# intel/oim

Hardware: AMD Instinct MI355X
Metric: 4KiB_randread_IOPS (higher is better)
Workload: dtype uint8

## Files before the change

native/include/hipstore/engine.h:

```cpp

#pragma once

#include <cstdint>
#include <functional>
#include <map>
#include <string>
#include <vector>

#include "hipstore/bdev.h"

namespace hipstore {

bool gpu_available();
int gpu_device_count();
std::string gpu_pci_address(int device);

BdevPtr create_hbm_bdev(const std::string& name, uint64_t block_size,
                        uint64_t num_blocks, int device,
                        bool persistent = false);

uint64_t persistent_stat(int which);

std::map<std::string, long long> persistent_probe(int device, int flags);

std::map<std::string, long long> persistent_kernel_probe(int device,
                                                         int variant);

std::pair<uint64_t, uint64_t> hbm_info(int device);

void* alloc_pinned(size_t bytes);
void free_pinned(void* ptr);

int hbm_copy_sync(Bdev* src, uint64_t src_offset, Bdev* dst,
                  uint64_t dst_offset, uint64_t length);

struct DiffStats {
  uint64_t granules = 0;
  uint64_t mismatched = 0;
  std::vector<uint64_t> first_mismatches;
};
int bdev_diff_sync(Bdev* a, uint64_t a_offset, Bdev* b, uint64_t b_offset,
                   uint64_t length, uint32_t granule, uint32_t max_report,
                   std::vector<uint64_t>* bitmap_out, DiffStats* stats);

uint64_t bdev_common_length(Bdev* a, uint64_t a_offset, Bdev* b,
                            uint64_t b_offset, uint32_t granule);

int bdev_copy_marked_sync(Bdev* src, uint64_t src_offset, Bdev* dst,
                          uint64_t dst_offset, uint64_t length,
                          uint32_t granule,
                          const std::vector<uint64_t>& bitmap,
                          uint64_t* copied = nullptr);

using PackSink =
    std::function<int(const uint8_t* data, uint64_t first_rank, uint64_t count)>;
int bdev_pack_marked_sync(Bdev* src, uint64_t src_offset, uint64_t length,
                          uint32_t granule,
                          const std::vector<uint64_t>& bitmap,
                          uint64_t staging_bytes, const PackSink& sink,
                          uint64_t* packed = nullptr);

using UnpackSource =
    std::function<int(uint8_t* data, uint64_t first_rank, uint64_t count)>;
int bdev_unpack_marked_sync(Bdev* dst, uint64_t dst_offset, uint64_t length,
// ... 16 lines not shown
  uint64_t granules = 0;
  uint64_t calls = 0;
};
int marked_copy_probe(Bdev* src, uint32_t granule,
                      const std::vector<uint64_t>& bitmap, int mode,
                      uint64_t ring_bytes, uint64_t staging_bytes,
                      MarkedCopyProbe* out);

int bdev_read_sync(Bdev* bdev, uint64_t offset, void* buf, uint64_t len);
int bdev_write_sync(Bdev* bdev, uint64_t offset, const void* buf, uint64_t len);
int bdev_fill_sync(Bdev* bdev, uint64_t offset, uint8_t value, uint64_t len);

class IoQueue {
 public:
  struct Op {
    IoOp op = IoOp::kRead;
    uint64_t offset = 0;
    uint64_t length = 0;
    uint8_t fill = 0;
    std::string payload;
  };
  struct Result {
    int status = kIoFailed;
    bool has_data = false;
    std::string data;
  };

  explicit IoQueue(BdevPtr bdev);

  const char* kind() const;

  std::vector<Result> run(const std::vector<Op>& ops);

  ~IoQueue();
  IoQueue(const IoQueue&) = delete;
  IoQueue& operator=(const IoQueue&) = delete;

 private:
  uint8_t* acquire_arena(uint64_t bytes);

  BdevPtr bdev_;
  std::shared_ptr<IoChannel> channel_;
  uint8_t* arena_ = nullptr;
  uint64_t arena_capacity_ = 0;
  std::vector<void*> retired_;
  bool busy_ = false;
};

struct PerfResult {
  double seconds = 0;
  uint64_t io_count = 0;
  double iops = 0;
  double throughput_mbps = 0;
  double lat_avg_us = 0;
  double lat_p50_us = 0;
  double lat_p90_us = 0;
  double lat_p99_us = 0;
  double lat_p999_us = 0;
  double lat_max_us = 0;
};

PerfResult run_bdevperf(Bdev* bdev, const std::string& workload,
                        uint32_t io_size, uint32_t queue_depth,
                        int num_queues, double seconds,
                        uint64_t max_ios = 0);

class PerfSession {
 public:
  PerfSession(BdevPtr bdev, std::string workload, uint32_t io_size,
              uint32_t queue_depth, int num_queues);
  ~PerfSession();

  PerfResult step(uint64_t total_ios);

 private:
  struct Impl;
  std::unique_ptr<Impl> impl_;
};

// ... 2 lines not shown
```

native/src/gpu.hip:

```cpp

#include <hip/hip_runtime.h>
#include <pthread.h>
#include <sched.h>
#include <unistd.h>
#include <stdlib.h>

#include <algorithm>
#include <atomic>
#include <chrono>
#include <condition_variable>
#include <cstring>
#include <deque>
#include <functional>
#include <map>
#include <mutex>
#include <random>
#include <set>
#include <stdexcept>
#include <thread>
#include <utility>
#include <vector>

#include "gpu_internal.h"
#include "hipstore/engine.h"

namespace hipstore {


namespace {

constexpr uint32_t kTileBytes = 4096;
constexpr uint32_t kRingSlots = 1 << 16;
constexpr uint32_t kMaxBatchTiles = kRingSlots / 4;

struct BlockDesc {
  const uint8_t* src;
  uint8_t* dst;
  uint32_t bytes;
  uint32_t fill;
};
static_assert(sizeof(BlockDesc) == 24, "persistent engine reads 3 x u64");

__global__ __launch_bounds__(kWavesPerWg * 64) void k_copy_blocks(
    const BlockDesc* __restrict__ descs, uint32_t n) {
  __shared__ __attribute__((aligned(16))) uint8_t lds_raw[kWavesPerWg * kTileBytes];
  const uint32_t wave = threadIdx.x >> 6;
  const uint32_t lane = threadIdx.x & 63;
  const uint32_t idx = blockIdx.x * kWavesPerWg + wave;
  if (idx >= n) return;
  const BlockDesc d = descs[idx];
  float4* lds = reinterpret_cast<float4*>(lds_raw + wave * kTileBytes);
  const uint32_t n16 = d.bytes >> 4;
  if (d.src != nullptr) {
    const float4* __restrict__ src = reinterpret_cast<const float4*>(d.src);
#pragma unroll 4
    for (uint32_t i = lane; i < n16; i += 64) lds[i] = src[i];
  } else {
// ... 446 lines not shown
  if (hipDeviceGetPCIBusId(bus_id, sizeof(bus_id), device) != hipSuccess) {
    return "";
  }
  std::string s(bus_id);
  std::transform(s.begin(), s.end(), s.begin(), ::tolower);
  return s;
}

std::pair<uint64_t, uint64_t> hbm_info(int device) {
  if (!gpu_available() || device < 0 || device >= gpu_device_count()) {
    return {0, 0};
  }
  if (hipSetDevice(device) != hipSuccess) return {0, 0};
  size_t free_bytes = 0;
  size_t total_bytes = 0;
  if (hipMemGetInfo(&free_bytes, &total_bytes) != hipSuccess) return {0, 0};
  return {total_bytes, free_bytes};
}

void* alloc_pinned(size_t bytes) {
  if (!gpu_available()) return malloc(bytes);
  void* p = nullptr;
  HIP_CHECK(hipHostMalloc(&p, bytes, hipHostMallocMapped));
  return p;
}

void free_pinned(void* ptr) {
  if (ptr == nullptr) return;
  if (!gpu_available()) {
    free(ptr);
    return;
  }
  (void)hipHostFree(ptr);
}


namespace {

class HbmChannelBase : public IoChannel {
 public:
  virtual void enqueue(IoRequest req, int status) = 0;
  virtual int poll() = 0;
  virtual const char* kind_name() const = 0;
};

inline HbmChannelBase* hbm_channel(IoChannel* ch) {
  return static_cast<HbmChannelBase*>(ch);
}

uint8_t* buf_device(uint8_t* host) {
  void* dev = nullptr;
  hipError_t err = hipHostGetDevicePointer(&dev, host, 0);
  if (err != hipSuccess) {
    throw std::runtime_error(
        "hipstore: I/O buffer is not pinned host memory (use alloc_pinned)");
  }
  return static_cast<uint8_t*>(dev);
}

inline uint32_t tile_count(uint64_t length) {
  return static_cast<uint32_t>((length + kTileBytes - 1) / kTileBytes);
}

void fill_desc(BlockDesc& d, const IoRequest& req, uint8_t* base,
               uint64_t done, uint32_t bytes) {
  if (req.op == IoOp::kRead) {
    d.src = base + req.offset + done;
    d.dst = buf_device(static_cast<uint8_t*>(req.buffer) + done);
  } else if (req.op == IoOp::kWrite) {
    d.src = buf_device(static_cast<uint8_t*>(req.buffer) + done);
    d.dst = base + req.offset + done;
  } else {
    d.src = nullptr;
    d.dst = base + req.offset + done;
  }
  d.bytes = bytes;
  d.fill = req.fill;
}

struct PendingIo {
  IoRequest req;
  int status;
};

struct InflightBatch {
  hipEvent_t event = nullptr;
  uint32_t slots = 0;
  std::vector<std::pair<IoCompletion, int>> completions;
};

class HbmChannel : public HbmChannelBase {
 public:
  HbmChannel(int device, uint8_t* base, uint64_t size)
      : base_(base), size_(size) {
    HIP_CHECK(hipSetDevice(device));
    HIP_CHECK(hipStreamCreateWithFlags(&stream_, hipStreamNonBlocking));
    HIP_CHECK(hipHostMalloc(reinterpret_cast<void**>(&ring_),
                            kRingSlots * sizeof(BlockDesc), hipHostMallocMapped));
    ring_dev_ = device_view(ring_);
    device_ = device;
  }

  ~HbmChannel() override {
// ... 56 lines not shown
    if (n > 0) {
      const uint32_t first = ring_head_;
      const uint32_t grid = (n + kWavesPerWg - 1) / kWavesPerWg;
      hipLaunchKernelGGL(k_copy_blocks, dim3(grid), dim3(kWavesPerWg * 64), 0,
                         stream_, ring_dev_ + first, n);
    }
    hipEvent_t event = get_event();
    HIP_CHECK(hipEventRecord(event, stream_));
    ring_head_ = (ring_head_ + n) % kRingSlots;
    used_slots_ += n;
    inflight_.push_back(InflightBatch{event, n, std::move(completions)});
  }

  int retire(bool wait) {
    int completed = 0;
    while (!inflight_.empty()) {
      InflightBatch& batch = inflight_.front();
      hipError_t st = wait ? hipEventSynchronize(batch.event)
                           : hipEventQuery(batch.event);
      if (st == hipErrorNotReady) break;
      if (st != hipSuccess) throw std::runtime_error("hip event failure");
      for (auto& [cb, status] : batch.completions) {
        if (cb) cb(status);
        ++completed;
      }
      used_slots_ -= batch.slots;
      event_pool_.push_back(batch.event);
      inflight_.pop_front();
    }
    return completed;
  }

  void expand(const IoRequest& req, uint32_t* slot) {
    uint64_t done = 0;
    while (done < req.length) {
      const uint32_t bytes = static_cast<uint32_t>(
          std::min<uint64_t>(kTileBytes, req.length - done));
      fill_desc(ring_[*slot], req, base_, done, bytes);
      ++*slot;
      done += bytes;
    }
  }

  hipEvent_t get_event() {
    if (!event_pool_.empty()) {
      hipEvent_t e = event_pool_.back();
      event_pool_.pop_back();
      return e;
    }
    hipEvent_t e = nullptr;
    HIP_CHECK(hipEventCreateWithFlags(&e, hipEventDisableTiming));
    return e;
  }

  uint8_t* base_;
  [[maybe_unused]] uint64_t size_;
  int device_ = 0;
  hipStream_t stream_ = nullptr;
  BlockDesc* ring_ = nullptr;
  BlockDesc* ring_dev_ = nullptr;
  uint32_t ring_head_ = 0;
  uint32_t used_slots_ = 0;
  std::vector<PendingIo> pending_;
  std::deque<InflightBatch> inflight_;
  std::vector<hipEvent_t> event_pool_;
};

class ServiceRingChannel : public HbmChannelBase {
 public:
  static constexpr uint32_t kRing = 32768;

  void enqueue(IoRequest req, int status) override {
    if (status != kIoOk) {
      immediate_.emplace_back(std::move(req.on_complete), status);
      return;
    }
    if (req.op == IoOp::kFlush) {
      flushes_.push_back({tail_, std::move(req.on_complete)});
      return;
    }
    pending_.push_back(std::move(req));
    drain_pending();
  }

  int poll() override {
    int completed = 0;
    if (!immediate_.empty()) {
      auto batch = std::move(immediate_);
      immediate_.clear();
      for (auto& [cb, status] : batch) {
        if (cb) cb(status);
        ++completed;
      }
    }
    const uint64_t retired_from = completed_;
    while (completed_ < tail_) {
// ... 54 lines not shown
    (void)hipHostFree(sq_);
    (void)hipHostFree(const_cast<unsigned long long*>(sq_tail_));
    (void)hipHostFree(const_cast<unsigned long long*>(cq_));
  }

  void delete_unfired() {
    std::set<IoState*> leftovers(desc_io_.begin(), desc_io_.end());
    for (IoState* state : leftovers) delete state;
  }

  BlockDesc* sq_ = nullptr;
  volatile unsigned long long* sq_tail_ = nullptr;
  volatile unsigned long long* cq_ = nullptr;
  uint64_t tail_ = 0;
  uint64_t completed_ = 0;
  std::chrono::steady_clock::time_point last_progress_{};

 private:
  struct IoState {
    IoCompletion cb;
    uint32_t remaining;
    int status;
  };

  bool has_capacity(uint32_t tiles) const {
    return tail_ - completed_ + tiles <= kRing;
  }

  void drain_pending() {
    while (!pending_.empty()) {
      IoRequest& req = pending_.front();
      const uint32_t tiles = tile_count(req.length);
      if (!has_capacity(tiles)) return;
      auto* state = new IoState{std::move(req.on_complete), tiles, kIoOk};
      uint64_t done = 0;
      uint64_t t = tail_;
      while (done < req.length) {
        const uint32_t bytes = static_cast<uint32_t>(
            std::min<uint64_t>(kTileBytes, req.length - done));
        fill_desc(sq_[t % kRing], req, base_, done, bytes);
        desc_io_[t % kRing] = state;
        ++t;
        done += bytes;
      }
      tail_ = t;
      __atomic_store_n(const_cast<unsigned long long*>(sq_tail_), tail_,
                       __ATOMIC_RELEASE);
      pending_.pop_front();
    }
  }

  uint8_t* base_;
  std::vector<IoState*> desc_io_;
  std::deque<IoRequest> pending_;
  std::deque<std::pair<uint64_t, IoCompletion>> flushes_;
  std::vector<std::pair<IoCompletion, int>> immediate_;
};

inline std::atomic<int> g_per_queue_channels[64];
inline int per_queue_channel_cap() {
  static const int cap = [] {
    const char* env = getenv("HIPSTORE_PERQ_CAP");
    return env ? atoi(env) : 18;
  }();
  return cap;
}

inline bool fallback_is_shared() {
  static const bool shared = [] {
    const char* env = getenv("HIPSTORE_FALLBACK");
    return env == nullptr || strcmp(env, "batched") != 0;
  }();
  return shared;
}

inline uint32_t batch_tiles_env() {
  const char* env = getenv("HIPSTORE_BATCH_TILES");
  const int v = env ? atoi(env) : 2;
  return static_cast<uint32_t>(
      std::min(std::max(v, 1), static_cast<int>(kMaxRunTiles)));
}

class HbmPersistentChannel : public ServiceRingChannel {
 public:
  static constexpr uint32_t kIdleSpins = 500000;

// ... 568 lines not shown
  req.fill = value;
  return run_sync(bdev, std::move(req));
}


IoQueue::IoQueue(BdevPtr bdev)
    : bdev_(std::move(bdev)), channel_(bdev_->get_channel()) {}

const char* IoQueue::kind() const {
  if (bdev_->device_base() == nullptr) return "cpu";
  return hbm_channel(channel_.get())->kind_name();
}

std::vector<IoQueue::Result> IoQueue::run(const std::vector<Op>& ops) {
  constexpr uint64_t kAlign = 64;
  std::vector<uint64_t> region(ops.size(), 0);
  uint64_t arena_bytes = kAlign;
  for (size_t i = 0; i < ops.size(); ++i) {
    if (ops[i].op != IoOp::kRead && ops[i].op != IoOp::kWrite) continue;
    region[i] = arena_bytes;
    arena_bytes += (ops[i].length + kAlign - 1) / kAlign * kAlign + kAlign;
  }
  uint8_t* arena = acquire_arena(arena_bytes);
  for (size_t i = 0; i < ops.size(); ++i) {
    if (ops[i].op == IoOp::kWrite && ops[i].length > 0) {
      memcpy(arena + region[i], ops[i].payload.data(), ops[i].length);
    } else if (ops[i].op == IoOp::kRead) {
      memset(arena + region[i], 0xDB, ops[i].length);
    }
  }

  struct RunState {
    std::vector<int> status;
    size_t remaining = 0;
  };
  auto state = std::make_shared<RunState>();
  state->status.assign(ops.size(), kIoFailed);
  state->remaining = ops.size();

  busy_ = true;
  for (size_t i = 0; i < ops.size(); ++i) {
    IoRequest req;
    req.op = ops[i].op;
    req.offset = ops[i].offset;
    req.length = ops[i].length;
    req.fill = ops[i].fill;
    if (req.op == IoOp::kRead || req.op == IoOp::kWrite) {
      req.buffer = arena + region[i];
    }
    req.on_complete = [state, i](int status) {
      state->status[i] = status;
      --state->remaining;
    };
    bdev_->submit(channel_.get(), std::move(req));
  }
  const auto deadline = std::chrono::steady_clock::now() +
                        std::chrono::duration<double>(sync_io_timeout_s());
  while (state->remaining > 0) {
    bdev_->poll(channel_.get());
    if (state->remaining > 0 &&
        std::chrono::steady_clock::now() > deadline) {
      dump_engine_stats("IoQueue timeout");
      throw std::runtime_error(
          "IoQueue: " + std::to_string(state->remaining) + " of " +
          std::to_string(ops.size()) + " requests still outstanding after " +
          std::to_string(sync_io_timeout_s()) + " s");
    }
  }

  std::vector<Result> results(ops.size());
  for (size_t i = 0; i < ops.size(); ++i) {
    results[i].status = state->status[i];
    if (ops[i].op == IoOp::kRead && state->status[i] == kIoOk) {
      results[i].has_data = true;
      results[i].data.assign(reinterpret_cast<const char*>(arena + region[i]),
                             ops[i].length);
    }
  }
  busy_ = false;
  return results;
}

uint8_t* IoQueue::acquire_arena(uint64_t bytes) {
  if (busy_) {
    arena_ = nullptr;
    arena_capacity_ = 0;
    retired_.clear();
    busy_ = false;
  }
  if (bytes > arena_capacity_) {
    if (arena_ != nullptr) retired_.push_back(arena_);
    arena_ = nullptr;
    arena_capacity_ = 0;
    void* p = alloc_pinned(bytes);
    if (p == nullptr) throw std::runtime_error("IoQueue: arena allocation");
    arena_ = static_cast<uint8_t*>(p);
    arena_capacity_ = bytes;
  }
  return arena_;
}

IoQueue::~IoQueue() {
  channel_.reset();
  if (busy_) return;
  for (void* p : retired_) free_pinned(p);
  free_pinned(arena_);
}


namespace {

struct LatHist {
// ... 361 lines not shown
  im.cv.notify_all();
  {
    const auto step_deadline =
        std::chrono::duration<double>(2 * sync_io_timeout_s() + 30.0);
    std::unique_lock<std::mutex> lock(im.mutex);
    const bool done = im.cv.wait_for(lock, step_deadline, [&] {
      for (auto& st : im.stats) {
        if (st.done_epoch < this_epoch) return false;
      }
      return true;
    });
    if (!done) {
      dump_engine_stats("perf-session step timeout");
      throw std::runtime_error("perf session: step timed out (wedged queue)");
    }
  }
  const double elapsed = std::chrono::duration<double>(clock::now() - t0).count();

  PerfResult result;
  result.seconds = elapsed;
  LatHist total;
  bool failed = false;
  for (auto& st : im.stats) {
    result.io_count += st.ios;
    failed |= st.failed;
    st.lat.merge_into(total);
  }
  if (failed) throw std::runtime_error("perf session: I/O failures");
  result.iops = result.io_count / elapsed;
  result.throughput_mbps =
      result.io_count * static_cast<double>(im.io_size) / elapsed / 1e6;
  total.fill_result(&result);
  return result;
}

std::map<std::string, long long> persistent_probe(int device, int flags) {
  std::map<std::string, long long> r;
  const bool use_atomics = flags & 1;
  const bool pre_memcpy = flags & 2;
  const bool do_rmw = flags & 4;
  const bool big_grid = flags & 8;
  const bool do_fence = flags & 16;
  r["flags"] = flags;
  HIP_CHECK(hipSetDevice(device));
  hipStream_t stream = nullptr;
  hipStream_t util = nullptr;
  HIP_CHECK(hipStreamCreateWithFlags(&stream, hipStreamNonBlocking));
  HIP_CHECK(hipStreamCreateWithFlags(&util, hipStreamNonBlocking));
  void* p_tail = nullptr;
  void* p_hb = nullptr;
  void* p_cq = nullptr;
  HIP_CHECK(hipHostMalloc(&p_tail, 8, hipHostMallocMapped));
  HIP_CHECK(hipHostMalloc(&p_hb, 8, hipHostMallocMapped));
  HIP_CHECK(hipHostMalloc(&p_cq, 16, hipHostMallocMapped));
  auto* tail = static_cast<volatile unsigned long long*>(p_tail);
  auto* hb = static_cast<volatile unsigned long long*>(p_hb);
  auto* cq = static_cast<volatile unsigned long long*>(p_cq);
  *tail = 0;
  *hb = 0;
  cq[0] = 0;
  cq[1] = 0;
  unsigned long long* dev_words = nullptr;
  HIP_CHECK(hipMalloc(reinterpret_cast<void**>(&dev_words), 24));
  HIP_CHECK(hipMemset(dev_words, 0, 24));
  HIP_CHECK(hipStreamSynchronize(nullptr));
  ProbeCtl ctl;
// ... 178 lines not shown
```

native/src/pybind.cpp:

```cpp

#include <pybind11/functional.h>
#include <pybind11/pybind11.h>
#include <pybind11/stl.h>

#include <cstring>
#include <optional>
#include <stdexcept>

#include "hipstore/bdev.h"
#include "hipstore/composite.h"
#include "hipstore/crc32c.h"
#include "hipstore/delta.h"
#include "hipstore/engine.h"
#include "hipstore/fingerprint.h"
#include "hipstore/nvmf.h"
#include "hipstore/rados.h"
#include "hipstore/vhost_master.h"

namespace py = pybind11;
using namespace hipstore;

namespace {

py::bytes bdev_read_py(Bdev& bdev, uint64_t offset, uint64_t length) {
  void* bounce = alloc_pinned(length);
  int status = bdev_read_sync(&bdev, offset, bounce, length);
  if (status != kIoOk) {
    free_pinned(bounce);
    throw std::runtime_error("bdev read failed: status " + std::to_string(status));
  }
  py::bytes out(static_cast<const char*>(bounce), length);
  free_pinned(bounce);
  return out;
}

void bdev_write_py(Bdev& bdev, uint64_t offset, py::buffer data) {
  py::buffer_info info = data.request();
  const uint64_t length = static_cast<uint64_t>(info.size) * info.itemsize;
  void* bounce = alloc_pinned(length);
  memcpy(bounce, info.ptr, length);
  int status = bdev_write_sync(&bdev, offset, bounce, length);
  free_pinned(bounce);
  if (status != kIoOk) {
    throw std::runtime_error("bdev write failed: status " + std::to_string(status));
  }
}

void bdev_fill_py(Bdev& bdev, uint64_t offset, int value, uint64_t length) {
  int status = bdev_fill_sync(&bdev, offset, static_cast<uint8_t>(value), length);
  if (status != kIoOk) {
    throw std::runtime_error("bdev fill failed: status " + std::to_string(status));
  }
}

IoQueue::Op io_op_from_tuple(const py::tuple& t) {
  if (t.empty()) throw std::invalid_argument("IoQueue: empty op tuple");
  const std::string name = t[0].cast<std::string>();
  IoQueue::Op op;
  if (name == "read" && t.size() == 3) {
    op.op = IoOp::kRead;
    op.offset = t[1].cast<uint64_t>();
    op.length = t[2].cast<uint64_t>();
  } else if (name == "write" && t.size() == 3) {
    op.op = IoOp::kWrite;
    op.offset = t[1].cast<uint64_t>();
    py::buffer_info info = t[2].cast<py::buffer>().request();
    op.payload.assign(static_cast<const char*>(info.ptr),
                      static_cast<size_t>(info.size) * info.itemsize);
    op.length = op.payload.size();
  } else if (name == "fill" && t.size() == 4) {
    op.op = IoOp::kFill;
    op.offset = t[1].cast<uint64_t>();
    op.length = t[2].cast<uint64_t>();
    op.fill = static_cast<uint8_t>(t[3].cast<int>());
  } else if (name == "flush" && t.size() == 1) {
    op.op = IoOp::kFlush;
  } else {
    throw std::invalid_argument("IoQueue: unknown op tuple '" + name + "'");
// ... 105 lines not shown
  }
  if (status == kIoOk) return;
  const std::string text = std::string(what) + ": " + error + " (status " +
                           std::to_string(status) + ")";
  if (status == kIoInvalid) throw std::invalid_argument(text);
  throw std::runtime_error(text);
}

}

PYBIND11_MODULE(_hipstore, m) {
  m.doc() = "MI355X hipstore data-path core (HBM bdevs, LDS-staged block I/O)";

  m.def("gpu_available", &gpu_available);
  m.def("gpu_device_count", &gpu_device_count);
  m.def("gpu_pci_address", &gpu_pci_address, py::arg("device"));

  py::class_<Bdev, BdevPtr>(m, "Bdev")
      .def_property_readonly("name", &Bdev::name)
      .def_property_readonly("product_name", &Bdev::product_name)
      .def_property_readonly("uuid", &Bdev::uuid)
      .def_property_readonly("block_size", &Bdev::block_size)
      .def_property_readonly("num_blocks", &Bdev::num_blocks)
      .def_property_readonly("size_bytes", &Bdev::size_bytes)
      .def("resize",
           [](hipstore::Bdev& b, uint64_t num_blocks) {
             return b.resize(num_blocks);
           },
           py::arg("num_blocks"))
      .def("read", &bdev_read_py, py::arg("offset"), py::arg("length"),
           py::call_guard<py::gil_scoped_release>())
      .def("write", &bdev_write_py, py::arg("offset"), py::arg("data"))
      .def("fill", &bdev_fill_py, py::arg("offset"), py::arg("value"),
           py::arg("length"), py::call_guard<py::gil_scoped_release>());

  m.def("create_malloc_bdev", &create_malloc_bdev, py::arg("name"),
        py::arg("block_size"), py::arg("num_blocks"));
  m.def("create_hbm_bdev", &create_hbm_bdev, py::arg("name"),
        py::arg("block_size"), py::arg("num_blocks"), py::arg("device") = 0,
        py::arg("persistent") = false);
  m.def("create_file_bdev", &create_file_bdev, py::arg("name"),
        py::arg("path"), py::arg("block_size") = 512);
  m.def("create_striped_bdev", &create_striped_bdev, py::arg("name"),
        py::arg("children"), py::arg("stripe_size") = 131072);
  m.def("create_replicated_bdev", &create_replicated_bdev, py::arg("name"),
        py::arg("children"));

  py::class_<RadosCluster, std::shared_ptr<RadosCluster>>(m, "RadosCluster")
      .def("port", &RadosCluster::port)
      .def("object_count", &RadosCluster::object_count)
      .def("stop", &RadosCluster::stop,
           py::call_guard<py::gil_scoped_release>());
  m.def("start_rados_cluster", &start_rados_cluster, py::arg("port") = 0,
        py::arg("arena_mb") = 512, py::arg("use_hbm") = false,
        py::arg("device") = 0, py::arg("object_bytes") = 4ull << 20);
  m.def("create_rbd_bdev", &create_rbd_bdev, py::arg("name"),
        py::arg("mon_host"), py::arg("pool"), py::arg("image"),
        py::arg("block_size") = 512,
        py::arg("default_size_bytes") = 64ull << 20,
        py::arg("object_bytes") = 4ull << 20);

  py::class_<NvmfTcpTarget, std::shared_ptr<NvmfTcpTarget>>(m, "NvmfTcpTarget")
      .def_property_readonly("port", &NvmfTcpTarget::port)
      .def("add_namespace", &NvmfTcpTarget::add_namespace, py::arg("bdev"))
      .def("stop", &NvmfTcpTarget::stop,
           py::call_guard<py::gil_scoped_release>());
  m.def("start_nvmf_tcp_target", &start_nvmf_tcp_target,
// ... 19 lines not shown
        {
          py::gil_scoped_release release;
          r = s.run(total_ios, workload);
        }
        return perf_to_dict(r);
      }, py::arg("total_ios"), py::arg("workload") = "randread");

  m.def(
      "vhost_master_bench",
      [](const std::string& socket_path, const std::string& personality,
         int num_rings, int iodepth, uint32_t io_size,
         const std::string& workload, uint64_t total_ios,
         uint32_t block_size, uint64_t capacity_bytes) {
        PerfResult r;
        {
          py::gil_scoped_release release;
          r = vhost_master_bench(socket_path, personality, num_rings,
                                 iodepth, io_size, workload, total_ios,
                                 block_size, capacity_bytes);
        }
        return perf_to_dict(r);
      },
      py::arg("socket_path"), py::arg("personality") = "scsi",
      py::arg("num_rings") = 4, py::arg("iodepth") = 32,
      py::arg("io_size") = 4096, py::arg("workload") = "randread",
      py::arg("total_ios") = 100000, py::arg("block_size") = 512,
      py::arg("capacity_bytes") = 0);

  py::class_<IoQueue>(m, "IoQueue",
                      "Queued I/O on one long-lived channel (tests): run() "
                      "submits every op before the first poll")
      .def(py::init<BdevPtr>(), py::arg("bdev"))
      .def_property_readonly("kind", &IoQueue::kind)
      .def("run", &io_queue_run_py, py::arg("ops"));

  py::class_<PerfSession>(m, "PerfSession")
      .def(py::init<BdevPtr, std::string, uint32_t, uint32_t, int>(),
           py::arg("bdev"), py::arg("workload") = "randread",
           py::arg("io_size") = 4096, py::arg("queue_depth") = 32,
           py::arg("num_queues") = 8)
      .def("step", [](PerfSession& s, uint64_t total_ios) {
        PerfResult r;
        {
          py::gil_scoped_release release;
          r = s.step(total_ios);
        }
        return perf_to_dict(r);
      }, py::arg("total_ios"));

  m.def(
      "run_bdevperf",
      [](BdevPtr bdev, const std::string& workload, uint32_t io_size,
         uint32_t queue_depth, int num_queues, double seconds,
         uint64_t max_ios) {
        PerfResult r;
        {
          py::gil_scoped_release release;
          r = run_bdevperf(bdev.get(), workload, io_size, queue_depth,
                           num_queues, seconds, max_ios);
        }
        return perf_to_dict(r);
      },
      py::arg("bdev"), py::arg("workload") = "randread",
      py::arg("io_size") = 4096, py::arg("queue_depth") = 32,
      py::arg("num_queues") = 1, py::arg("seconds") = 2.0,
      py::arg("max_ios") = 0);

  m.def("hbm_info", [](int device) {
    auto [total, free_bytes] = hbm_info(device);
    return py::make_tuple(total, free_bytes);
  }, py::arg("device") = 0);

  m.def("hbm_copy", [](BdevPtr src, uint64_t src_offset, BdevPtr dst,
                       uint64_t dst_offset, uint64_t length) {
    int status;
    {
      py::gil_scoped_release release;
      status = hbm_copy_sync(src.get(), src_offset, dst.get(), dst_offset,
                             length);
    }
    if (status != kIoOk) {
      throw std::runtime_error("hbm_copy failed: status " +
                               std::to_string(status));
    }
  }, py::arg("src"), py::arg("src_offset"), py::arg("dst"),
     py::arg("dst_offset"), py::arg("length"),
     "Device-side range copy between HBM bdevs (LDS-staged kernel "
     "same-device, xGMI peer copy cross-device)");

  m.def("bdev_diff", [](BdevPtr a, BdevPtr b, uint64_t a_offset,
                        uint64_t b_offset, uint64_t length, uint32_t granule,
                        uint32_t max_report) {
    if (granule == 0) granule = static_cast<uint32_t>(a->block_size());
    if (length == 0) length = bdev_common_length(a.get(), a_offset, b.get(),
                                                     b_offset, granule);
    std::vector<uint64_t> bitmap;
    DiffStats stats;
    int status;
    {
// ... 373 lines not shown
```

native/src/vhost.cpp:

```cpp

#include "hipstore/vhost.h"

#include <poll.h>
#include <sys/eventfd.h>
#include <sys/mman.h>
#include <sys/socket.h>
#include <sys/un.h>
#include <pthread.h>
#include <sched.h>
#include <unistd.h>

#include <hip/hip_runtime.h>

#include <cstring>
#include <map>
#include <mutex>
#include <set>
#include <stdexcept>
#include <thread>
#include <vector>

#include "hipstore/engine.h"

namespace hipstore {
// ... 478 lines not shown

  bool set_mem_table(Msg& msg) {
    unmap_regions();
    uint32_t nregions = 0;
    if (msg.payload.size() < 8) return false;
    memcpy(&nregions, msg.payload.data(), 4);
    if (nregions > kMaxRegions || msg.fds.size() < nregions ||
        msg.payload.size() < 8 + nregions * sizeof(MemRegionWire)) {
      return false;
    }
    for (uint32_t i = 0; i < nregions; ++i) {
      MemRegionWire w;
      memcpy(&w, msg.payload.data() + 8 + i * sizeof(w), sizeof(w));
      size_t maplen = w.memory_size + w.mmap_offset;
      void* map = ::mmap(nullptr, maplen, PROT_READ | PROT_WRITE, MAP_SHARED,
                         msg.fds[i], 0);
      ::close(msg.fds[i]);
      msg.fds[i] = -1;
      if (map == MAP_FAILED) {
        unmap_regions();
        return false;
      }
      Region region;
      region.gpa = w.guest_phys_addr;
      region.size = w.memory_size;
      region.uaddr = w.userspace_addr;
      region.map = static_cast<uint8_t*>(map);
      region.maplen = maplen;
      region.base = region.map + w.mmap_offset;
      if (gpu_available()) {
        region.hip_registered =
            hipHostRegister(region.base, region.size,
                            hipHostRegisterMapped) == hipSuccess;
      }
      regions_.push_back(region);
    }
    return true;
  }

  void unmap_regions() {
    for (const Region& r : regions_) {
      if (r.hip_registered) (void)hipHostUnregister(r.base);
      ::munmap(r.map, r.maplen);
    }
    regions_.clear();
  }

  uint8_t* gpa_to_ptr(uint64_t gpa, uint64_t len) {
    for (const Region& r : regions_) {
      if (gpa >= r.gpa && len <= r.size && gpa - r.gpa <= r.size - len) {
        return r.base + (gpa - r.gpa);
      }
    }
    return nullptr;
  }

  uint8_t* uaddr_to_ptr(uint64_t uaddr, uint64_t len) {
    for (const Region& r : regions_) {
      if (uaddr >= r.uaddr && len <= r.size &&
          uaddr - r.uaddr <= r.size - len) {
        return r.base + (uaddr - r.uaddr);
      }
    }
    return nullptr;
  }


  struct Vring {
    uint32_t num = 0;
    uint16_t last_avail = 0;
    uint16_t used_idx = 0;
    VringDesc* desc = nullptr;
    VringAvail* avail = nullptr;
    VringUsed* used = nullptr;
    int kick = -1;
// ... 969 lines not shown
```

Measured before the change: 12.70 million.

## Cache pinned host-to-device pointer translations per channel

Adds a small per-channel LRU cache of pinned host ranges, so each request resolves its device buffer pointer once instead of calling hipHostGetDevicePointer for every tile descriptor. Frees and unregistrations bump a global generation counter that invalidates the caches. Host-registered vhost regions are tracked and excluded from range caching. Also adds probe and test drivers plus completion-order tracking, at the cost of a mutex-guarded range check on cache misses.

```diff
diff --git a/native/include/hipstore/engine.h b/native/include/hipstore/engine.h
--- a/native/include/hipstore/engine.h
+++ b/native/include/hipstore/engine.h
@@ -30,6 +30,13 @@
 
 void* alloc_pinned(size_t bytes);
 void free_pinned(void* ptr);
+
+void pinned_ranges_changed();
+
+void note_host_registered(void* base, uint64_t size);
+void host_unregister(void* base);
+
+std::map<std::string, double> submit_path_probe(int threads, uint64_t iters);
 
 int hbm_copy_sync(Bdev* src, uint64_t src_offset, Bdev* dst,
                   uint64_t dst_offset, uint64_t length);
@@ -112,6 +119,8 @@
 
   std::vector<Result> run(const std::vector<Op>& ops);
 
+  const std::vector<uint32_t>& last_order() const { return last_order_; }
+
   ~IoQueue();
   IoQueue(const IoQueue&) = delete;
   IoQueue& operator=(const IoQueue&) = delete;
@@ -125,6 +134,7 @@
   uint64_t arena_capacity_ = 0;
   std::vector<void*> retired_;
   bool busy_ = false;
+  std::vector<uint32_t> last_order_;
 };
 
 struct PerfResult {
diff --git a/native/include/hipstore/pin_cache.h b/native/include/hipstore/pin_cache.h
--- /dev/null
+++ b/native/include/hipstore/pin_cache.h
@@ -0,0 +1,72 @@
+
+#pragma once
+
+#include <atomic>
+#include <cstdint>
+
+namespace hipstore {
+
+inline std::atomic<uint64_t> g_pinned_generation{0};
+
+inline uint64_t pinned_generation() {
+  return g_pinned_generation.load(std::memory_order_relaxed);
+}
+
+inline void bump_pinned_generation() {
+  g_pinned_generation.fetch_add(1, std::memory_order_release);
+}
+
+struct PinnedRange {
+  uintptr_t host_base = 0;
+  uint64_t size = 0;
+  uintptr_t dev_base = 0;
+
+  bool holds(uintptr_t p, uint64_t len) const {
+    return p >= host_base && len <= size && p - host_base <= size - len;
+  }
+};
+
+class PinTranslationCache {
+ public:
+  static constexpr int kEntries = 4;
+
+  template <typename Resolver>
+  uint8_t* translate(uint8_t* host, uint64_t len, Resolver&& resolve) {
+    const uint64_t generation = pinned_generation();
+    if (generation != generation_) {
+      count_ = 0;
+      generation_ = generation;
+    }
+    const uintptr_t p = reinterpret_cast<uintptr_t>(host);
+    for (int i = 0; i < count_; ++i) {
+      if (!entries_[i].holds(p, len)) continue;
+      const PinnedRange hit = entries_[i];
+      for (int k = i; k > 0; --k) entries_[k] = entries_[k - 1];
+      entries_[0] = hit;
+      ++hits_;
+      return reinterpret_cast<uint8_t*>(hit.dev_base + (p - hit.host_base));
+    }
+    ++misses_;
+    PinnedRange range;
+    uint8_t* dev = resolve(host, &range);
+    if (range.size != 0 && range.holds(p, len)) {
+      if (count_ < kEntries) ++count_;
+      for (int k = count_ - 1; k > 0; --k) entries_[k] = entries_[k - 1];
+      entries_[0] = range;
+    }
+    return dev;
+  }
+
+  int size() const { return count_; }
+  uint64_t hits() const { return hits_; }
+  uint64_t misses() const { return misses_; }
+
+ private:
+  PinnedRange entries_[kEntries];
+  int count_ = 0;
+  uint64_t generation_ = 0;
+  uint64_t hits_ = 0;
+  uint64_t misses_ = 0;
+};
+
+}
diff --git a/native/include/hipstore/submit_path_driver.h b/native/include/hipstore/submit_path_driver.h
--- /dev/null
+++ b/native/include/hipstore/submit_path_driver.h
@@ -0,0 +1,48 @@
+
+#pragma once
+
+#include <cstdint>
+#include <string>
+#include <vector>
+
+#include "hipstore/bdev.h"
+
+namespace hipstore {
+
+struct TwoBufferResult {
+  std::string pattern_a, pattern_b, pattern_c;
+  std::string final_a, final_b, final_c;
+  std::vector<int> status;
+  std::string pageable_error;
+  bool c_reused_a = false;
+};
+TwoBufferResult submit_path_two_buffers(const BdevPtr& bdev, uint32_t tiles);
+
+struct ResubmitResult {
+  uint64_t completed = 0;
+  uint64_t failed = 0;
+  bool in_order = true;
+};
+ResubmitResult submit_path_resubmit(const BdevPtr& bdev, uint64_t total,
+                                    uint32_t depth);
+
+struct IoStatSnapshot {
+  uint64_t num_read_ops = 0;
+  uint64_t num_write_ops = 0;
+  uint64_t num_unmap_ops = 0;
+  uint64_t bytes_read = 0;
+  uint64_t bytes_written = 0;
+};
+IoStatSnapshot iostat_snapshot(Bdev& bdev);
+
+struct StatsResult {
+  IoStatSnapshot before, after;
+  uint64_t samples = 0;
+  bool monotone = true;
+  uint64_t failed = 0;
+};
+StatsResult submit_path_stats(const BdevPtr& bdev, int threads,
+                              uint32_t reads, uint32_t writes,
+                              uint32_t fills);
+
+}
diff --git a/native/src/gpu.hip b/native/src/gpu.hip
--- a/native/src/gpu.hip
+++ b/native/src/gpu.hip
@@ -23,6 +23,7 @@
 
 #include "gpu_internal.h"
 #include "hipstore/engine.h"
+#include "hipstore/pin_cache.h"
 
 namespace hipstore {
 
@@ -535,6 +536,46 @@
     return;
   }
   (void)hipHostFree(ptr);
+  pinned_ranges_changed();
+}
+
+void pinned_ranges_changed() { bump_pinned_generation(); }
+
+namespace {
+
+std::mutex g_registered_mutex;
+std::vector<std::pair<uintptr_t, uint64_t>> g_registered_ranges;
+
+bool host_registered(const void* ptr) {
+  const uintptr_t p = reinterpret_cast<uintptr_t>(ptr);
+  std::lock_guard<std::mutex> lock(g_registered_mutex);
+  for (const auto& [base, size] : g_registered_ranges) {
+    if (p >= base && p - base < size) return true;
+  }
+  return false;
+}
+
+}
+
+void note_host_registered(void* base, uint64_t size) {
+  std::lock_guard<std::mutex> lock(g_registered_mutex);
+  g_registered_ranges.emplace_back(reinterpret_cast<uintptr_t>(base), size);
+}
+
+void host_unregister(void* base) {
+  (void)hipHostUnregister(base);
+  {
+    const uintptr_t p = reinterpret_cast<uintptr_t>(base);
+    std::lock_guard<std::mutex> lock(g_registered_mutex);
+    for (auto it = g_registered_ranges.begin();
+         it != g_registered_ranges.end(); ++it) {
+      if (it->first == p) {
+        g_registered_ranges.erase(it);
+        break;
+      }
+    }
+  }
+  pinned_ranges_changed();
 }
 
 
@@ -551,27 +592,54 @@
   return static_cast<HbmChannelBase*>(ch);
 }
 
-uint8_t* buf_device(uint8_t* host) {
+uint8_t* resolve_pinned(uint8_t* host, PinnedRange* range) {
   void* dev = nullptr;
   hipError_t err = hipHostGetDevicePointer(&dev, host, 0);
   if (err != hipSuccess) {
+    (void)hipGetLastError();
     throw std::runtime_error(
         "hipstore: I/O buffer is not pinned host memory (use alloc_pinned)");
   }
+  hipDeviceptr_t dev_base = nullptr;
+  size_t size = 0;
+  if (!host_registered(host) &&
+      hipMemGetAddressRange(&dev_base, &size, dev) == hipSuccess &&
+      dev_base != nullptr && size != 0) {
+    const uintptr_t d = reinterpret_cast<uintptr_t>(dev);
+    const uintptr_t db = reinterpret_cast<uintptr_t>(dev_base);
+    if (d >= db && d - db < size) {
+      uint8_t* host_base = host - (d - db);
+      void* check = nullptr;
+      if (hipHostGetDevicePointer(&check, host_base, 0) == hipSuccess &&
+          check == dev_base && !host_registered(host_base)) {
+        range->host_base = reinterpret_cast<uintptr_t>(host_base);
+        range->size = size;
+        range->dev_base = db;
+      }
+    }
+  }
+  if (range->size == 0) (void)hipGetLastError();
   return static_cast<uint8_t*>(dev);
+}
+
+inline uint8_t* request_buffer_device(PinTranslationCache& cache,
+                                      const IoRequest& req) {
+  if (req.op != IoOp::kRead && req.op != IoOp::kWrite) return nullptr;
+  return cache.translate(static_cast<uint8_t*>(req.buffer), req.length,
+                         resolve_pinned);
 }
 
 inline uint32_t tile_count(uint64_t length) {
   return static_cast<uint32_t>((length + kTileBytes - 1) / kTileBytes);
 }
 
-void fill_desc(BlockDesc& d, const IoRequest& req, uint8_t* base,
-               uint64_t done, uint32_t bytes) {
+inline void fill_desc(BlockDesc& d, const IoRequest& req, uint8_t* base,
+                      uint8_t* buf, uint64_t done, uint32_t bytes) {
   if (req.op == IoOp::kRead) {
     d.src = base + req.offset + done;
-    d.dst = buf_device(static_cast<uint8_t*>(req.buffer) + done);
+    d.dst = buf + done;
   } else if (req.op == IoOp::kWrite) {
-    d.src = buf_device(static_cast<uint8_t*>(req.buffer) + done);
+    d.src = buf + done;
     d.dst = base + req.offset + done;
   } else {
     d.src = nullptr;
@@ -694,11 +762,12 @@
   }
 
   void expand(const IoRequest& req, uint32_t* slot) {
+    uint8_t* buf = request_buffer_device(translations_, req);
     uint64_t done = 0;
     while (done < req.length) {
       const uint32_t bytes = static_cast<uint32_t>(
           std::min<uint64_t>(kTileBytes, req.length - done));
-      fill_desc(ring_[*slot], req, base_, done, bytes);
+      fill_desc(ring_[*slot], req, base_, buf, done, bytes);
       ++*slot;
       done += bytes;
     }
@@ -724,6 +793,7 @@
   uint32_t ring_head_ = 0;
   uint32_t used_slots_ = 0;
   std::vector<PendingIo> pending_;
+  PinTranslationCache translations_;
   std::deque<InflightBatch> inflight_;
   std::vector<hipEvent_t> event_pool_;
 };
@@ -844,13 +914,20 @@
       IoRequest& req = pending_.front();
       const uint32_t tiles = tile_count(req.length);
       if (!has_capacity(tiles)) return;
+      uint8_t* buf = nullptr;
+      try {
+        buf = request_buffer_device(translations_, req);
+      } catch (...) {
+        pending_.pop_front();
+        throw;
+      }
       auto* state = new IoState{std::move(req.on_complete), tiles, kIoOk};
       uint64_t done = 0;
       uint64_t t = tail_;
       while (done < req.length) {
         const uint32_t bytes = static_cast<uint32_t>(
             std::min<uint64_t>(kTileBytes, req.length - done));
-        fill_desc(sq_[t % kRing], req, base_, done, bytes);
+        fill_desc(sq_[t % kRing], req, base_, buf, done, bytes);
         desc_io_[t % kRing] = state;
         ++t;
         done += bytes;
@@ -864,6 +941,7 @@
 
   uint8_t* base_;
   std::vector<IoState*> desc_io_;
+  PinTranslationCache translations_;
   std::deque<IoRequest> pending_;
   std::deque<std::pair<uint64_t, IoCompletion>> flushes_;
   std::vector<std::pair<IoCompletion, int>> immediate_;
@@ -1498,6 +1576,7 @@
 
   struct RunState {
     std::vector<int> status;
+    std::vector<uint32_t> order;
     size_t remaining = 0;
   };
   auto state = std::make_shared<RunState>();
@@ -1516,6 +1595,7 @@
     }
     req.on_complete = [state, i](int status) {
       state->status[i] = status;
+      state->order.push_back(static_cast<uint32_t>(i));
       --state->remaining;
     };
     bdev_->submit(channel_.get(), std::move(req));
@@ -1544,6 +1624,7 @@
     }
   }
   busy_ = false;
+  last_order_ = std::move(state->order);
   return results;
 }
 
@@ -1971,6 +2052,91 @@
       result.io_count * static_cast<double>(im.io_size) / elapsed / 1e6;
   total.fill_result(&result);
   return result;
+}
+
+std::map<std::string, double> submit_path_probe(int threads,
+                                                uint64_t iters) {
+  using clock = std::chrono::steady_clock;
+  if (threads < 1 || threads > 64 || iters == 0) {
+    throw std::runtime_error("submit_path_probe: 1..64 threads, iters > 0");
+  }
+  if (!gpu_available()) {
+    throw std::runtime_error("submit_path_probe: no HIP device");
+  }
+  struct StatsOnlyBdev : Bdev {
+    StatsOnlyBdev() : Bdev("probe", "probe", 512, 8) {}
+    std::shared_ptr<IoChannel> get_channel() override { return nullptr; }
+    void submit(IoChannel*, IoRequest) override {}
+    int poll(IoChannel*) override { return 0; }
+  };
+  struct StateSized {
+    IoCompletion cb;
+    uint32_t remaining;
+    int status;
+  };
+  struct alignas(64) PrivateLine {
+    std::atomic<uint64_t> ops{0};
+    std::atomic<uint64_t> bytes{0};
+  };
+  auto shared = std::make_shared<StatsOnlyBdev>();
+  std::vector<PrivateLine> own(threads);
+  std::vector<void*> pinned(threads, nullptr);
+  for (auto& p : pinned) p = alloc_pinned(4096 * 32);
+
+  auto measure = [&](auto body) {
+    std::atomic<int> ready{0};
+    std::atomic<bool> go{false};
+    std::vector<double> ns(threads, 0);
+    std::vector<std::thread> pool;
+    for (int t = 0; t < threads; ++t) {
+      pool.emplace_back([&, t] {
+        maybe_pin_thread(t);
+        ready.fetch_add(1);
+        while (!go.load(std::memory_order_acquire)) __builtin_ia32_pause();
+        const auto t0 = clock::now();
+        for (uint64_t i = 0; i < iters; ++i) body(t, i);
+        ns[t] = std::chrono::duration<double, std::nano>(clock::now() - t0)
+                    .count() / static_cast<double>(iters);
+      });
+    }
+    while (ready.load() < threads) std::this_thread::yield();
+    go.store(true, std::memory_order_release);
+    for (auto& th : pool) th.join();
+    double sum = 0;
+    for (double v : ns) sum += v;
+    return sum / threads;
+  };
+
+  std::map<std::string, double> out;
+  std::atomic<uint64_t> sink{0};
+  out["get_device_pointer"] = measure([&](int t, uint64_t i) {
+    void* dev = nullptr;
+    (void)hipHostGetDevicePointer(
+        &dev, static_cast<uint8_t*>(pinned[t]) + (i & 31) * 4096, 0);
+    if (dev == nullptr) sink.fetch_add(1, std::memory_order_relaxed);
+  });
+  IoRequest req;
+  req.op = IoOp::kRead;
+  req.length = 4096;
+  out["iostat_shared"] =
+      measure([&](int, uint64_t) { shared->account(req); });
+  out["iostat_private"] = measure([&](int t, uint64_t) {
+    own[t].ops.fetch_add(1, std::memory_order_relaxed);
+    own[t].bytes.fetch_add(4096, std::memory_order_relaxed);
+  });
+  out["new_delete"] = measure([&](int, uint64_t i) {
+    auto* s = new StateSized{nullptr, static_cast<uint32_t>(i), 0};
+    StateSized* volatile keep = s;
+    delete keep;
+  });
+  out["clock_now"] = measure([&](int, uint64_t) {
+    volatile int64_t keep = clock::now().time_since_epoch().count();
+    (void)keep;
+  });
+  for (void* p : pinned) free_pinned(p);
+  out["checksum"] = static_cast<double>(
+      shared->iostat().num_read_ops.load() + own[0].ops.load() + sink.load());
+  return out;
 }
 
 std::map<std::string, long long> persistent_probe(int device, int flags) {
diff --git a/native/src/pybind.cpp b/native/src/pybind.cpp
--- a/native/src/pybind.cpp
+++ b/native/src/pybind.cpp
@@ -15,6 +15,7 @@
 #include "hipstore/fingerprint.h"
 #include "hipstore/nvmf.h"
 #include "hipstore/rados.h"
+#include "hipstore/submit_path_driver.h"
 #include "hipstore/vhost_master.h"
 
 namespace py = pybind11;
@@ -44,6 +45,16 @@
   if (status != kIoOk) {
     throw std::runtime_error("bdev write failed: status " + std::to_string(status));
   }
+}
+
+py::dict iostat_to_dict(const IoStatSnapshot& st) {
+  py::dict d;
+  d["num_read_ops"] = st.num_read_ops;
+  d["num_write_ops"] = st.num_write_ops;
+  d["num_unmap_ops"] = st.num_unmap_ops;
+  d["bytes_read"] = st.bytes_read;
+  d["bytes_written"] = st.bytes_written;
+  return d;
 }
 
 void bdev_fill_py(Bdev& bdev, uint64_t offset, int value, uint64_t length) {
@@ -215,7 +226,10 @@
            py::call_guard<py::gil_scoped_release>())
       .def("write", &bdev_write_py, py::arg("offset"), py::arg("data"))
       .def("fill", &bdev_fill_py, py::arg("offset"), py::arg("value"),
-           py::arg("length"), py::call_guard<py::gil_scoped_release>());
+           py::arg("length"), py::call_guard<py::gil_scoped_release>())
+      .def("iostat",
+           [](Bdev& b) { return iostat_to_dict(iostat_snapshot(b)); },
+           "the counters get_bdevs_iostat reports");
 
   m.def("create_malloc_bdev", &create_malloc_bdev, py::arg("name"),
         py::arg("block_size"), py::arg("num_blocks"));
@@ -301,7 +315,8 @@
                       "submits every op before the first poll")
       .def(py::init<BdevPtr>(), py::arg("bdev"))
       .def_property_readonly("kind", &IoQueue::kind)
-      .def("run", &io_queue_run_py, py::arg("ops"));
+      .def("run", &io_queue_run_py, py::arg("ops"))
+      .def_property_readonly("last_order", &IoQueue::last_order);
 
   py::class_<PerfSession>(m, "PerfSession")
       .def(py::init<BdevPtr, std::string, uint32_t, uint32_t, int>(),
@@ -334,6 +349,60 @@
       py::arg("io_size") = 4096, py::arg("queue_depth") = 32,
       py::arg("num_queues") = 1, py::arg("seconds") = 2.0,
       py::arg("max_ios") = 0);
+
+  m.def("submit_path_probe", &submit_path_probe, py::arg("threads"),
+        py::arg("iters") = 1000000,
+        py::call_guard<py::gil_scoped_release>(),
+        "ns per operation of the submit path's per-I/O suspects on "
+        "`threads` threads at once (no kernel launched)");
+
+  m.def("submit_path_two_buffers", [](BdevPtr bdev, uint32_t tiles) {
+    TwoBufferResult r;
+    {
+      py::gil_scoped_release release;
+      r = submit_path_two_buffers(bdev, tiles);
+    }
+    py::dict d;
+    d["pattern_a"] = py::bytes(r.pattern_a);
+    d["pattern_b"] = py::bytes(r.pattern_b);
+    d["pattern_c"] = py::bytes(r.pattern_c);
+    d["final_a"] = py::bytes(r.final_a);
+    d["final_b"] = py::bytes(r.final_b);
+    d["final_c"] = py::bytes(r.final_c);
+    d["status"] = r.status;
+    d["pageable_error"] = r.pageable_error;
+    d["c_reused_a"] = r.c_reused_a;
+    return d;
+  }, py::arg("bdev"), py::arg("tiles") = 4);
+  m.def("submit_path_resubmit", [](BdevPtr bdev, uint64_t total,
+                                   uint32_t depth) {
+    ResubmitResult r;
+    {
+      py::gil_scoped_release release;
+      r = submit_path_resubmit(bdev, total, depth);
+    }
+    py::dict d;
+    d["completed"] = r.completed;
+    d["failed"] = r.failed;
+    d["in_order"] = r.in_order;
+    return d;
+  }, py::arg("bdev"), py::arg("total"), py::arg("depth") = 32);
+  m.def("submit_path_stats", [](BdevPtr bdev, int threads, uint32_t reads,
+                                uint32_t writes, uint32_t fills) {
+    StatsResult r;
+    {
+      py::gil_scoped_release release;
+      r = submit_path_stats(bdev, threads, reads, writes, fills);
+    }
+    py::dict d;
+    d["before"] = iostat_to_dict(r.before);
+    d["after"] = iostat_to_dict(r.after);
+    d["samples"] = r.samples;
+    d["monotone"] = r.monotone;
+    d["failed"] = r.failed;
+    return d;
+  }, py::arg("bdev"), py::arg("threads"), py::arg("reads"),
+     py::arg("writes"), py::arg("fills"));
 
   m.def("hbm_info", [](int device) {
     auto [total, free_bytes] = hbm_info(device);
diff --git a/native/src/submit_path_driver.cpp b/native/src/submit_path_driver.cpp
--- /dev/null
+++ b/native/src/submit_path_driver.cpp
@@ -0,0 +1,281 @@
+
+#include "hipstore/submit_path_driver.h"
+
+#include <atomic>
+#include <chrono>
+#include <cstdlib>
+#include <cstring>
+#include <memory>
+#include <stdexcept>
+#include <thread>
+
+#include "hipstore/engine.h"
+
+namespace hipstore {
+
+namespace {
+
+constexpr uint64_t kTile = 4096;
+constexpr double kWaitSeconds = 30.0;
+
+void poll_until_done(Bdev* bdev, IoChannel* ch,
+                     const std::shared_ptr<uint64_t>& remaining) {
+  const auto deadline = std::chrono::steady_clock::now() +
+                        std::chrono::duration<double>(kWaitSeconds);
+  uint32_t polls = 0;
+  while (*remaining > 0) {
+    bdev->poll(ch);
+    if ((++polls & 0x3FF) == 0 &&
+        std::chrono::steady_clock::now() > deadline) {
+      throw std::runtime_error("submit-path driver: " +
+                               std::to_string(*remaining) +
+                               " requests still outstanding");
+    }
+  }
+}
+
+struct Step {
+  IoOp op;
+  uint64_t offset;
+  uint8_t* buffer;
+};
+
+void run_steps(Bdev* bdev, IoChannel* ch, const std::vector<Step>& steps,
+               std::vector<int>* status) {
+  auto remaining = std::make_shared<uint64_t>(steps.size());
+  auto results = std::make_shared<std::vector<int>>(steps.size(), kIoFailed);
+  for (size_t i = 0; i < steps.size(); ++i) {
+    IoRequest req;
+    req.op = steps[i].op;
+    req.offset = steps[i].offset;
+    req.length = kTile;
+    req.buffer = steps[i].buffer;
+    req.on_complete = [remaining, results, i](int st) {
+      (*results)[i] = st;
+      --*remaining;
+    };
+    bdev->submit(ch, std::move(req));
+  }
+  poll_until_done(bdev, ch, remaining);
+  status->insert(status->end(), results->begin(), results->end());
+}
+
+std::string make_pattern(uint64_t bytes, uint32_t mul, uint32_t add) {
+  std::string s(bytes, '\0');
+  for (uint64_t i = 0; i < bytes; ++i) {
+    s[i] = static_cast<char>((i * mul + add + (i >> 8)) & 0xFF);
+  }
+  return s;
+}
+
+}
+
+IoStatSnapshot iostat_snapshot(Bdev& bdev) {
+  Bdev::IoStat& st = bdev.iostat();
+  IoStatSnapshot s;
+  s.num_read_ops = st.num_read_ops.load(std::memory_order_relaxed);
+  s.num_write_ops = st.num_write_ops.load(std::memory_order_relaxed);
+  s.num_unmap_ops = st.num_unmap_ops.load(std::memory_order_relaxed);
+  s.bytes_read = st.bytes_read.load(std::memory_order_relaxed);
+  s.bytes_written = st.bytes_written.load(std::memory_order_relaxed);
+  return s;
+}
+
+TwoBufferResult submit_path_two_buffers(const BdevPtr& bdev, uint32_t tiles) {
+  if (tiles < 2) throw std::runtime_error("two_buffers: at least 2 tiles");
+  const uint64_t bytes = tiles * kTile;
+  const uint64_t last = (tiles - 1) * kTile;
+  TwoBufferResult out;
+  out.pattern_a = make_pattern(bytes, 7, 1);
+  out.pattern_b = make_pattern(bytes, 13, 5);
+  out.pattern_c = make_pattern(bytes, 29, 11);
+
+  auto channel = bdev->get_channel();
+  IoChannel* ch = channel.get();
+  auto* a = static_cast<uint8_t*>(alloc_pinned(bytes));
+  auto* b = static_cast<uint8_t*>(alloc_pinned(bytes));
+  memcpy(a, out.pattern_a.data(), bytes);
+  memcpy(b, out.pattern_b.data(), bytes);
+  run_steps(bdev.get(), ch,
+            {{IoOp::kWrite, 0 * kTile, a},
+             {IoOp::kWrite, 1 * kTile, b},
+             {IoOp::kWrite, 2 * kTile, a + last},
+             {IoOp::kWrite, 3 * kTile, b + last}},
+            &out.status);
+  memset(a, 0, bytes);
+  memset(b, 0, bytes);
+  run_steps(bdev.get(), ch,
+            {{IoOp::kRead, 0 * kTile, b + last},
+             {IoOp::kRead, 1 * kTile, a + last},
+             {IoOp::kRead, 2 * kTile, b},
+             {IoOp::kRead, 3 * kTile, a}},
+            &out.status);
+  out.final_a.assign(reinterpret_cast<char*>(a), bytes);
+  out.final_b.assign(reinterpret_cast<char*>(b), bytes);
+
+  free_pinned(a);
+  auto* c = static_cast<uint8_t*>(alloc_pinned(bytes));
+  out.c_reused_a = c == a;
+  memcpy(c, out.pattern_c.data(), bytes);
+  run_steps(bdev.get(), ch,
+            {{IoOp::kWrite, 4 * kTile, c}, {IoOp::kWrite, 5 * kTile, c + last}},
+            &out.status);
+  memset(c, 0, bytes);
+  run_steps(bdev.get(), ch,
+            {{IoOp::kRead, 4 * kTile, c + last}, {IoOp::kRead, 5 * kTile, c}},
+            &out.status);
+  out.final_c.assign(reinterpret_cast<char*>(c), bytes);
+
+  void* pageable = nullptr;
+  if (posix_memalign(&pageable, 4096, kTile) != 0) {
+    throw std::runtime_error("two_buffers: posix_memalign");
+  }
+  try {
+    std::vector<int> ignored;
+    run_steps(bdev.get(), ch,
+              {{IoOp::kRead, 0, static_cast<uint8_t*>(pageable)}}, &ignored);
+    out.pageable_error = "(accepted)";
+  } catch (const std::exception& e) {
+    out.pageable_error = e.what();
+  }
+  channel.reset();
+  free(pageable);
+  free_pinned(b);
+  free_pinned(c);
+  return out;
+}
+
+ResubmitResult submit_path_resubmit(const BdevPtr& bdev, uint64_t total,
+                                    uint32_t depth) {
+  const uint64_t units = bdev->size_bytes() / kTile;
+  if (units == 0 || depth == 0 || units < 2ull * depth) {
+    throw std::runtime_error("resubmit: bdev too small for the depth");
+  }
+  struct Run {
+    Bdev* bdev = nullptr;
+    IoChannel* ch = nullptr;
+    uint8_t* buf = nullptr;
+    uint64_t total = 0;
+    uint64_t units = 0;
+    uint64_t submitted = 0;
+    uint64_t next_expected = 0;
+    ResubmitResult result;
+
+    void submit(uint32_t slot) {
+      const uint64_t i = submitted++;
+      auto* words = reinterpret_cast<uint64_t*>(buf + slot * kTile);
+      for (uint64_t k = 0; k < kTile / 8; ++k) {
+        words[k] = i * 0x9E3779B97F4A7C15ull + k;
+      }
+      IoRequest req;
+      req.op = IoOp::kWrite;
+      req.offset = (i % units) * kTile;
+      req.length = kTile;
+      req.buffer = buf + slot * kTile;
+      req.on_complete = [this, slot, i](int status) {
+        if (status != kIoOk) ++result.failed;
+        if (i != next_expected) result.in_order = false;
+        next_expected = i + 1;
+        ++result.completed;
+        if (submitted < total) submit(slot);
+      };
+      bdev->submit(ch, std::move(req));
+    }
+  };
+  auto run = std::make_shared<Run>();
+  auto channel = bdev->get_channel();
+  run->bdev = bdev.get();
+  run->ch = channel.get();
+  run->buf = static_cast<uint8_t*>(alloc_pinned(depth * kTile));
+  run->total = total;
+  run->units = units;
+  const uint32_t initial =
+      static_cast<uint32_t>(std::min<uint64_t>(depth, total));
+  for (uint32_t slot = 0; slot < initial; ++slot) run->submit(slot);
+  const auto deadline = std::chrono::steady_clock::now() +
+                        std::chrono::duration<double>(kWaitSeconds);
+  uint32_t polls = 0;
+  while (run->result.completed < total) {
+    bdev->poll(run->ch);
+    if ((++polls & 0x3FF) == 0 &&
+        std::chrono::steady_clock::now() > deadline) {
+      new std::shared_ptr<Run>(run);
+      throw std::runtime_error("resubmit: requests still outstanding");
+    }
+  }
+  channel.reset();
+  free_pinned(run->buf);
+  return run->result;
+}
+
+StatsResult submit_path_stats(const BdevPtr& bdev, int threads,
+                              uint32_t reads, uint32_t writes,
+                              uint32_t fills) {
+  StatsResult out;
+  const uint64_t region = bdev->size_bytes() / threads;
+  if (threads < 1 || region < 65536) {
+    throw std::runtime_error("stats: bdev too small for the threads");
+  }
+  out.before = iostat_snapshot(*bdev);
+  std::atomic<int> running{threads};
+  std::atomic<uint64_t> failed{0};
+  std::vector<std::thread> pool;
+  for (int t = 0; t < threads; ++t) {
+    pool.emplace_back([&, t] {
+      try {
+        auto channel = bdev->get_channel();
+        auto* buf = static_cast<uint8_t*>(alloc_pinned(8192));
+        memset(buf, 0x40 + t, 8192);
+        const uint64_t base = t * region;
+        uint32_t left[3] = {reads, writes, fills};
+        const uint64_t length[3] = {512ull * (t + 1), 4096, 8192};
+        const IoOp op[3] = {IoOp::kRead, IoOp::kWrite, IoOp::kFill};
+        uint64_t n = 0;
+        while (left[0] + left[1] + left[2] > 0) {
+          const int kind = static_cast<int>(n % 3);
+          ++n;
+          if (left[kind] == 0) continue;
+          --left[kind];
+          auto remaining = std::make_shared<uint64_t>(1);
+          IoRequest req;
+          req.op = op[kind];
+          req.offset = base + (n % 4) * 8192;
+          req.length = length[kind];
+          req.buffer = kind == 2 ? nullptr : buf;
+          req.fill = static_cast<uint8_t>(t);
+          req.on_complete = [remaining, &failed](int status) {
+            if (status != kIoOk) failed.fetch_add(1);
+            --*remaining;
+          };
+          bdev->submit(channel.get(), std::move(req));
+          poll_until_done(bdev.get(), channel.get(), remaining);
+        }
+        channel.reset();
+        free_pinned(buf);
+      } catch (const std::exception&) {
+        failed.fetch_add(1u << 20);
+      }
+      running.fetch_sub(1);
+    });
+  }
+  IoStatSnapshot prev = out.before;
+  while (running.load() > 0) {
+    const IoStatSnapshot now = iostat_snapshot(*bdev);
+    if (now.num_read_ops < prev.num_read_ops ||
+        now.num_write_ops < prev.num_write_ops ||
+        now.num_unmap_ops < prev.num_unmap_ops ||
+        now.bytes_read < prev.bytes_read ||
+        now.bytes_written < prev.bytes_written) {
+      out.monotone = false;
+    }
+    prev = now;
+    ++out.samples;
+    std::this_thread::yield();
+  }
+  for (auto& th : pool) th.join();
+  out.after = iostat_snapshot(*bdev);
+  out.failed = failed.load();
+  return out;
+}
+
+}
diff --git a/native/src/vhost.cpp b/native/src/vhost.cpp
--- a/native/src/vhost.cpp
+++ b/native/src/vhost.cpp
@@ -534,6 +534,9 @@
         region.hip_registered =
             hipHostRegister(region.base, region.size,
                             hipHostRegisterMapped) == hipSuccess;
+        if (region.hip_registered) {
+          note_host_registered(region.base, region.size);
+        }
       }
       regions_.push_back(region);
     }
@@ -542,7 +545,7 @@
 
   void unmap_regions() {
     for (const Region& r : regions_) {
-      if (r.hip_registered) (void)hipHostUnregister(r.base);
+      if (r.hip_registered) host_unregister(r.base);
       ::munmap(r.map, r.maplen);
     }
     regions_.clear();
```

Result: no change. 12.65 million, median of 2 (-0.4%).
